# Mingrui-Yu/A-Simple-Stereo-SLAM-System-with-Deep-Loop-Closing

Measured on AMD Instinct MI355X. Metric: stereo frames/sec (ORB+match+LCD+BA-build) @1241x376, higher is better.
Workload: dtype u8/int32 (ORB, Hamming), f32 via f16x3 / bf16x6 split products on the matrix cores with f32 accumulate (CALC conv1 / conv2, DB scan), f64 (triangulation, BA)

## Files before the change

### a-simple-stereo-slam-system-with-deep-loop-closing_amd/csrc/orb_engine.hip

```cpp
#include <math.h>
#include <stdlib.h>
#include <string.h>

#include <vector>

#include "common.h"
#include "orb_plan.h"

namespace myslam_hip {

void launch_resize(const ResizeArgs& a, int batch, hipStream_t s);
void launch_resize_chain(const ResizeArgs* lv, int n, int batch, hipStream_t s);
bool resize_is_little(const ResizeArgs& a, int batch);
int resize_chain_max();
int pyr_head_levels();
void launch_pyr_head(const ResizeArgs* lv, int n, int rows, int cols, uint8_t* dst0, int dpitch0, size_t dstride0, int b0, int batch,
                     uint32_t* p0, int n0, uint32_t* p1, int n1, uint32_t* p2, int n2, uint32_t* p3, int n3, hipStream_t s);
void launch_blur(const BlurArgs& a, int batch, hipStream_t s);
bool blur_uses_strips(const BlurArgs& a);
bool resize_uses_strips(const ResizeArgs& a);
void launch_fast(const OrbPlan& P, const uint8_t* pyr, size_t pyrStride, const uint8_t* maskPyr, uint32_t* cand,
                 int32_t* candCount, const uint32_t* statPrev, uint32_t* statCur, int forceMode, int batch, hipStream_t s);
bool launch_octree(const OrbPlan& P, const uint32_t* cand, const int32_t* candCount, uint32_t* sortbuf, const uint32_t* octTab, uint32_t* selOut,
                   int32_t* selCount, int32_t* status, int batch, uint16_t* order, hipStream_t s, const BlurArgs* blurLv, int nBlur);
bool describe_uses_tile_order(bool have_order, int detectOnly, int batch);
void launch_describe(const OrbPlan& P, const uint8_t* pyr, const uint8_t* blur, size_t pyrStride, const uint32_t* selOut,
                     const int32_t* selCount, myslam_keypoint* kps, uint8_t* desc, int32_t* counts, int32_t* status,
                     int cap, int detectOnly, int batch, uint16_t* order, bool order_ready, int blocks_per_cu, hipStream_t s);
void launch_screen(const OrbPlan& P, const uint8_t* pyr, myslam_keypoint* kin, int n, myslam_keypoint* kout, uint8_t* keep,
                   hipStream_t s);
void launch_calc_desc(const OrbPlan& P, const uint8_t* blur, const myslam_keypoint* kps, int n, uint8_t* desc, hipStream_t s);
void launch_unpack_cands(const uint32_t* cand, int n, int32_t* xs, int32_t* ys, int32_t* sc, hipStream_t s);
void launch_blur_levels(const BlurArgs* lv, int n, int batch, hipStream_t s);
bool blur_mfma_tables(int w, int h, const int q[7], std::vector<uint4>& tab, size_t& offH, size_t& offV);
void blur_mfma_ident(std::vector<uint4>& tab, size_t& offI);
void launch_zero_u32(uint32_t* p0, int n0, uint32_t* p1, int n1, uint32_t* p2, int n2, uint32_t* p3, int n3, hipStream_t s);
void launch_ingest_clear(const uint8_t* src, int rows, int cols, int step, size_t sstride, uint8_t* dst, int dpitch, size_t dstride, int batch,
                         uint32_t* p0, int n0, uint32_t* p1, int n1, uint32_t* p2, int n2, uint32_t* p3, int n3, hipStream_t s);
void launch_ingest(const uint8_t* src, int rows, int cols, int step, size_t sstride, uint8_t* dst, int dpitch,
                   size_t dstride, int batch, hipStream_t s);
// ... 33 lines not shown
    MYSLAM_HIP_CHECK(hipMalloc((void**)&p, n * sizeof(T)));
    return MYSLAM_OK;
}

}

using namespace myslam_hip;

struct myslam_orb {
    int nfeatures, nlevels, iniTh, minTh;
    float scaleFactor;
    std::vector<float> scale, invScale;
    std::vector<int> nPerLevel;
    int umax[16];
    hipStream_t stream = nullptr;
    hipStream_t aux = nullptr;
    hipEvent_t evFork = nullptr, evJoin = nullptr;
    hipEvent_t evUserFast = nullptr;
    hipEvent_t evUserGate = nullptr;

    int rows = 0, cols = 0;
    OrbPlan full{}, det{};

    int batchCap = 0;
    bool maskAlloc = false;
    uint8_t *d_pyr = nullptr, *d_blur = nullptr, *d_mask = nullptr;
    uint32_t* d_cand = nullptr;
    uint32_t* d_sort = nullptr;
    int32_t *d_candCount = nullptr, *d_selCount = nullptr, *d_status = nullptr;
    uint32_t* d_sel = nullptr;
    uint16_t* d_order = nullptr;
    uint32_t* d_octTab = nullptr;
    uint32_t* d_stripTab = nullptr;
    uint32_t* d_fastStat = nullptr; int fastFlip = 0;
    int optFastMode = -1;
    int optInternalStream = 1;
    int optCopyInput = 0;
    int optStopAfter = 0;
    int tapsSet = 0, taps[7] = {0};
    int optSideBlocksPerCu = 0;
    int optBlurMfma = 0;
    uint4* d_blurTab = nullptr; bool blurTabValid = false; size_t blurOffI = 0, blurOffH[MAXL] = {0}, blurOffV[MAXL] = {0}; bool blurLvOk[MAXL] = {false}; int blurVconst = 0;
    int ensure_blur_tables();

    struct HostGraph { hipGraphExec_t exec = nullptr; hipGraph_t graph = nullptr; uint64_t gen = 0; int rows = 0, cols = 0, step = 0, dcap = 0, calls = 0; bool mask = false; };
    HostGraph hostGraph[2][2];
    uint64_t gen = 1;
    struct Clear { uint32_t* p[4]; int n[4]; } clr{{nullptr, nullptr, nullptr, nullptr}, {0, 0, 0, 0}};
    hipStream_t hostStream = nullptr;
    uint8_t* h_pin = nullptr; size_t pinBytes = 0;
    int ensure_pin(size_t bytes);
    void drop_host_graphs();
    uint8_t *d_stageImg = nullptr, *d_stageMask = nullptr; size_t stageImgBytes = 0, stageMaskBytes = 0;
    myslam_keypoint *d_stageKps = nullptr, *d_stageKps2 = nullptr; uint8_t* d_stageDesc = nullptr; uint8_t* d_stageKeep = nullptr;
    int32_t* d_stageCounts = nullptr; int stageCap = 0;
    uint8_t* d_stageOut = nullptr; size_t stageOutBytes = 0, stageDescOff = 0;

    int make_tables();
    int make_plan(int r, int c);
    int ensure(int batch, int r, int c, bool needMask);
    int ensure_stage(size_t imgBytes, size_t maskBytes, int cap);
    int build_pyramids(const uint8_t* d_imgs, int batch, int step, size_t stride, const uint8_t* d_masks, int nlev);
    ResizeArgs level_resize_args(uint8_t* base, int l) const;
    BlurArgs level_blur_args(int l) const;
    int blur_levels(int batch, int nlev, hipStream_t s);
    void fill_blur_args(BlurArgs* lv, int nlev) const;
// ... 109 lines not shown
            const int spr = (g.nCols + 3) / 4;
            for (int strip = 0; strip < g.nRows * spr; strip++) {
                uint32_t* e = st.data() + (size_t)(g.stripBase + strip) * 8;
                const int ci = strip / spr, cj0 = (strip - ci * spr) * 4;
                const int iniY = MIN_BORDER + ci * g.hCell;
                int ncell = 0, pairs = 0; uint32_t wcs = 0; int hr = 0;
                if (iniY < g.maxBY - 3) {
                    hr = std::min(iniY + g.hCell + 6, g.maxBY) - iniY;
                    const int hc = hr - 6;
                    if (hc > 0)
                        for (int c = 0; c < 4; c++) {
                            const int cj = cj0 + c, iniX = MIN_BORDER + cj * g.wCell;
                            int wc = 0;
                            if (cj < g.nCols && iniX < g.maxBX - 6) wc = std::max(0, std::min(iniX + g.wCell + 6, g.maxBX) - iniX - 6);
                            if (wc > 0) ncell = c + 1;
                            wcs |= (uint32_t)wc << (8 * c);
                            pairs += ((wc + 1) >> 1) * hc;
                        }
                }
                if (ncell == 0) wcs = 0;
                e[0] = (uint32_t)l | ((uint32_t)ci << 8) | ((uint32_t)cj0 << 16) | ((uint32_t)ncell << 24);
                e[1] = (uint32_t)iniY | ((uint32_t)hr << 16);
                e[2] = (uint32_t)(MIN_BORDER + cj0 * g.wCell) | ((uint32_t)g.wCell << 16);
                e[3] = wcs; e[4] = (uint32_t)g.pitch; e[5] = (uint32_t)pairs;
                e[6] = (uint32_t)(g.imgOff & 0xffffffffu); e[7] = (uint32_t)(g.imgOff >> 32);
            }
        }
        int rc = dev_alloc(d_stripTab, st.size());
        if (rc) return rc;
        if ((rc = upload_table(d_stripTab, st.data(), st.size() * sizeof(uint32_t)))) return rc;
        P.stripTab = d_stripTab;
    }
    full = P;
    det = P;
    det.nlevels = 1;
    det.ncells = P.lv[0].nCols * P.lv[0].nRows;
    det.nstrips = P.lv[0].nRows * ((P.lv[0].nCols + 3) / 4);
    det.lv[0].N = nfeatures;
    det.lv[0].nodeCap = (std::max(nfeatures + 4, 4 * P.lv[0].nIni + 4) + 3) & ~3;
    if (det.lv[0].nodeCap > 4092) return MYSLAM_ERR_UNSUPPORTED;
    det.lv[0].outBase = 0;
    det.totalOut = det.lv[0].nodeCap;
    rows = r; cols = c;
    return MYSLAM_OK;
}

int myslam_orb::ensure(int batch, int r, int c, bool needMask) {
    if (r != rows || c != cols) {
        MYSLAM_HIP_CHECK(hipStreamSynchronize(stream));
        int rc = make_plan(r, c);
        if (rc) { rows = cols = 0; return rc; }
        batchCap = 0; gen++; blurTabValid = false;
    }
    const int detOut = det.totalOut;
    const size_t selPer = (size_t)std::max(full.totalOut, detOut);
    if (batch > batchCap) {
        MYSLAM_HIP_CHECK(hipStreamSynchronize(stream));
        gen++;
        int rc;
        if ((rc = dev_alloc(d_pyr, (size_t)batch * full.pyrBytes + 64))) return rc;
        if ((rc = dev_alloc(d_blur, (size_t)batch * full.pyrBytes + 4096))) return rc;
        if ((rc = dev_alloc(d_cand, (size_t)batch * full.totalKeyCap))) return rc;
        if ((rc = dev_alloc(d_sort, (size_t)batch * full.totalKeyCap * 2))) return rc;
        if ((rc = dev_alloc(d_candCount, (size_t)batch * MAXL))) return rc;
        if ((rc = dev_alloc(d_selCount, (size_t)batch * MAXL))) return rc;
        if ((rc = dev_alloc(d_status, (size_t)batch))) return rc;
// ... 40 lines not shown
                launch_ingest(src + (size_t)n0 * stride, P.rows, P.cols, step, stride, dst0, P.lv[0].pitch, P.pyrBytes, batch - n0, stream);
            }
        }
        for (; l < nlev;) {
            ScopedProf sp(P_RESIZE, stream);
            ResizeArgs a = level_resize_args(base, l);
            if (l == 1 && n0 > 0) { a.src0 = d_imgs; a.spitch0 = step; a.sstride0 = stride; a.n0 = n0; }
            ResizeArgs grp[4]; int ng = 0;
            const int gmax = resize_chain_max();
            if (gmax > 1 && resize_is_little(a, batch)) {
                static const double kEvals[4] = {1, 5, 21, 85};
                double evals = (double)batch * a.dw * a.dh;
                grp[ng++] = a;
                while (ng < gmax && l + ng < nlev) {
                    const ResizeArgs nx = level_resize_args(base, l + ng);
                    evals += (double)batch * nx.dw * nx.dh * kEvals[ng];
                    if (!resize_is_little(nx, batch) || evals > 6e6) break;
                    grp[ng++] = nx;
                }
            }
            if (ng > 1) { launch_resize_chain(grp, ng, batch, stream); l += ng; }
            else { launch_resize(a, batch, stream); l++; }
        }
    }
    return MYSLAM_OK;
}
ResizeArgs myslam_orb::level_resize_args(uint8_t* base, int l) const {
    const OrbPlan& P = full;
    ResizeArgs a;
    a.src = base + P.lv[l - 1].imgOff; a.sw = P.lv[l - 1].w; a.sh = P.lv[l - 1].h; a.spitch = P.lv[l - 1].pitch; a.sstride = P.pyrBytes;
    a.src0 = nullptr; a.spitch0 = 0; a.n0 = 0; a.sstride0 = 0;
    a.dst = base + P.lv[l].imgOff; a.dw = P.lv[l].w; a.dh = P.lv[l].h; a.dpitch = P.lv[l].pitch; a.dstride = P.pyrBytes;
    a.scale_x = 1. / ((double)a.dw / a.sw); a.scale_y = 1. / ((double)a.dh / a.sh);
    return a;
}
int myslam_orb::ensure_blur_tables() {
    if (blurTabValid) return MYSLAM_OK;
    std::vector<uint4> tab;
    int q[7];
    if (tapsSet) memcpy(q, taps, sizeof(q)); else gauss_q8(0, q);
    int sum = 0;
    for (int t = 0; t < 7; t++) sum += q[t];
    blurVconst = sum * 128 * sum + 32768;
    blur_mfma_ident(tab, blurOffI);
    for (int l = 0; l < full.nlevels; l++) blurLvOk[l] = blur_mfma_tables(full.lv[l].w, full.lv[l].h, q, tab, blurOffH[l], blurOffV[l]);
    MYSLAM_HIP_CHECK(hipStreamSynchronize(stream));
    int rc = dev_alloc(d_blurTab, tab.size());
    if (rc) return rc;
    if ((rc = upload_table(d_blurTab, tab.data(), tab.size() * sizeof(uint4)))) return rc;
    blurTabValid = true; gen++;
    return MYSLAM_OK;
}

BlurArgs myslam_orb::level_blur_args(int l) const {
    const OrbPlan& P = full;
    BlurArgs a;
    a.src = d_pyr + P.lv[l].imgOff; a.dst = d_blur + P.lv[l].imgOff;
    a.w = P.lv[l].w; a.h = P.lv[l].h; a.spitch = a.dpitch = P.lv[l].pitch; a.sstride = a.dstride = P.pyrBytes;
    a.src0 = nullptr; a.spitch0 = 0; a.n0 = 0; a.sstride0 = 0;
    a.dtiled = 1;
    if (tapsSet) memcpy(a.q, taps, sizeof(taps)); else gauss_q8(0, a.q);
    if (optBlurMfma && blurTabValid && blurLvOk[l]) { a.tabH = d_blurTab + blurOffH[l]; a.tabV = d_blurTab + blurOffV[l]; a.ident = d_blurTab + blurOffI; a.vconst = blurVconst; }
    return a;
}
void myslam_orb::fill_blur_args(BlurArgs* lv, int nlev) const {
    const OrbPlan& P = full;
// ... 102 lines not shown
    if (h_pin) { (void)hipHostFree(h_pin); h_pin = nullptr; pinBytes = 0; }
    gen++;
    const size_t want = (bytes + (bytes >> 2) + 4095) & ~(size_t)4095;
    MYSLAM_HIP_CHECK(hipHostMalloc((void**)&h_pin, want));
    pinBytes = want;
    return MYSLAM_OK;
}

void myslam_orb::drop_host_graphs() {
    for (auto& row : hostGraph)
        for (auto& g : row) { if (g.exec) (void)hipGraphExecDestroy(g.exec); if (g.graph) (void)hipGraphDestroy(g.graph); g = HostGraph(); }
}

int myslam_orb::ensure_stage(size_t imgBytes, size_t maskBytes, int cap) {
    if (imgBytes > stageImgBytes) { gen++; int rc = dev_alloc(d_stageImg, imgBytes); if (rc) return rc; stageImgBytes = imgBytes; }
    if (maskBytes > stageMaskBytes) { gen++; int rc = dev_alloc(d_stageMask, maskBytes); if (rc) return rc; stageMaskBytes = maskBytes; }
    if (cap > stageCap) {
        gen++;
        int rc;
        const size_t oK = 256, oD = oK + (((size_t)cap * sizeof(myslam_keypoint) + 255) & ~(size_t)255), total = oD + (size_t)cap * 32;
        if ((rc = dev_alloc(d_stageOut, total))) return rc;
        stageOutBytes = total; stageDescOff = oD;
        d_stageCounts = reinterpret_cast<int32_t*>(d_stageOut);
        d_stageKps = reinterpret_cast<myslam_keypoint*>(d_stageOut + oK);
        d_stageDesc = d_stageOut + oD;
        if ((rc = dev_alloc(d_stageKps2, (size_t)cap))) return rc;
        if ((rc = dev_alloc(d_stageKeep, (size_t)cap))) return rc;
        stageCap = cap;
    }
    return MYSLAM_OK;
}

void myslam_orb::free_all() {
    void* ptrs[] = {d_blurTab, d_fastStat, d_octTab, d_stripTab, d_pyr, d_blur, d_mask, d_cand, d_sort, d_candCount, d_selCount, d_status, d_sel, d_order, d_stageImg, d_stageMask,
                    d_stageOut, d_stageKps2, d_stageKeep};
    for (void* p : ptrs) if (p) (void)hipFree(p);
    if (aux) { (void)hipStreamSynchronize(aux); (void)hipStreamDestroy(aux); (void)hipEventDestroy(evFork); (void)hipEventDestroy(evJoin); aux = nullptr; }
    drop_host_graphs();
    if (hostStream) { (void)hipStreamSynchronize(hostStream); (void)hipStreamDestroy(hostStream); hostStream = nullptr; }
    if (h_pin) { (void)hipHostFree(h_pin); h_pin = nullptr; pinBytes = 0; }
}

extern "C" {

int myslam_orb_create(myslam_orb** out, int nfeatures, float scale_factor, int nlevels, int ini_th_fast, int min_th_fast) {
    if (!out || nfeatures < 1 || nlevels < 1 || nlevels > MAXL || !(scale_factor > 1.0f) || ini_th_fast < 0 ||
        min_th_fast < 1 || min_th_fast > ini_th_fast || ini_th_fast > 255 || scale_factor > 2.5f)
        return MYSLAM_ERR_INVALID;
    int ndev = 0;
    if (hipGetDeviceCount(&ndev) != hipSuccess || ndev < 1) return MYSLAM_ERR_HIP;
    myslam_orb* h = new myslam_orb();
    h->nfeatures = nfeatures; h->scaleFactor = scale_factor; h->nlevels = nlevels; h->iniTh = ini_th_fast; h->minTh = min_th_fast;
    int rc = h->make_tables();
    if (rc) { delete h; return rc; }
    *out = h;
    return MYSLAM_OK;
}

int myslam_orb_destroy(myslam_orb* h) {
    if (!h) return MYSLAM_ERR_INVALID;
    (void)hipStreamSynchronize(h->stream);
    h->free_all();
    delete h;
    return MYSLAM_OK;
}

int myslam_orb_set_stream(myslam_orb* h, void* s) {
// ... 334 lines not shown
```

### a-simple-stereo-slam-system-with-deep-loop-closing_amd/csrc/orb_kernels.hip

```cpp
#include <stdio.h>
#include <stdlib.h>

#include <type_traits>

#include "common.h"
#include "orb_plan.h"

namespace myslam_hip {

typedef unsigned short u16x2 __attribute__((ext_vector_type(2)));

#ifdef MYSLAM_BLOCK_TRACE
__device__ unsigned long long* g_bt_buf = nullptr;
__device__ unsigned int g_bt_cap = 0, g_bt_n = 0;
struct BlockTrace {
    unsigned long long t0 = 0, marks = 0, aux = 0; int kid; unsigned hw = 0; bool on = false;
    __device__ __forceinline__ void mark(int i) {
        if (on) marks |= ((__builtin_amdgcn_s_memrealtime() - t0) & 0xffffull) << (16 * i);
    }
    __device__ __forceinline__ BlockTrace(int kid_) : kid(kid_) {
        if (threadIdx.x != 0 || g_bt_buf == nullptr) return;
        const unsigned xcc = __builtin_amdgcn_s_getreg((3 << 11) | 20) & 0xf;
        if (xcc != 0) return;
        hw = __builtin_amdgcn_s_getreg((31 << 11) | 4);
// ... 113 lines not shown
        return min(max(v, 0), 255);
    }
}

__host__ __device__ constexpr int rc_px(int J) { return J >= 4 ? 1 : 4; }

template <int J>
__device__ __forceinline__ void rc_store(const ResizeChain& c, const uint8_t* S, uint8_t* D, int item) {
    const int dw = c.dw[J - 1], dh = c.dh[J - 1], gpr = (dw + 3) >> 2;
    if constexpr (rc_px(J) == 4) {
        const int dy = item / gpr, dx4 = (item - dy * gpr) * 4;
        if (dy >= dh) return;
        uint32_t packed = 0;
#pragma unroll
        for (int k = 0; k < 4; k++) packed |= (uint32_t)rc_pix<J>(c, S, min(dx4 + k, dw - 1), dy) << (8 * k);
        *reinterpret_cast<uint32_t*>(D + (size_t)dy * c.dpitch[J - 1] + dx4) = packed;
    } else {
        const int dy = item / (4 * gpr), dx = item - dy * 4 * gpr;
        if (dy >= dh) return;
        D[(size_t)dy * c.dpitch[J - 1] + dx] = (uint8_t)rc_pix<J>(c, S, min(dx, dw - 1), dy);
    }
}

__device__ __forceinline__ void rc_block(const ResizeChain& c, int blk, int b) {
    const uint8_t* S = c.src + (size_t)b * c.sstride;
    if (blk < c.blk0[1]) rc_store<1>(c, S, c.dst[0] + (size_t)b * c.dstride, blk * 256 + (int)threadIdx.x);
    else if (blk < c.blk0[2]) rc_store<2>(c, S, c.dst[1] + (size_t)b * c.dstride, (blk - c.blk0[1]) * 256 + (int)threadIdx.x);
    else if (blk < c.blk0[3]) rc_store<3>(c, S, c.dst[2] + (size_t)b * c.dstride, (blk - c.blk0[2]) * 256 + (int)threadIdx.x);
    else rc_store<4>(c, S, c.dst[3] + (size_t)b * c.dstride, (blk - c.blk0[3]) * 256 + (int)threadIdx.x);
}

__global__ __launch_bounds__(256) void k_resize_chain(ResizeChain c) { rc_block(c, blockIdx.x, blockIdx.y); }

constexpr int RS_R = 8;
constexpr int RS_NB = 2;
constexpr int RS_MAXR = 12;

__global__ __launch_bounds__(256) void k_resize_strip(ResizeArgs a, int nstrips, int nbands) {
    MYSLAM_SIDE_PRIO();
    MYSLAM_BT(1);
    const int lane = threadIdx.x & 63;
    const int wid = __builtin_amdgcn_readfirstlane((int)(blockIdx.x * 4 + (threadIdx.x >> 6)));
    const int ngroups = (nbands + RS_NB - 1) / RS_NB;
    if (wid >= nstrips * ngroups) return;
    const int strip = wid % nstrips, group = wid / nstrips;
    const int b = blockIdx.z;
    const int dx4 = strip * 256 + 4 * lane;
    const bool has = dx4 < a.dw;
    const bool ext = b < a.n0;
    const uint8_t* src = ext ? a.src0 + (size_t)b * a.sstride0 : a.src + (size_t)b * a.sstride;
    const int spitch = ext ? a.spitch0 : a.spitch;
    uint8_t* dst = a.dst + (size_t)b * a.dstride;
    int sx[4]; uint32_t aw[4];
#pragma unroll
    for (int k = 0; k < 4; k++) {
        int c0, c1;
        resize_coord(min(dx4 + k, a.dw - 1), a.scale_x, a.sw, true, sx[k], c0, c1);
        aw[k] = (uint32_t)c0 | ((uint32_t)c1 << 16);
    }
    uint32_t selk[4];
#pragma unroll
    for (int k = 0; k < 4; k++) { const uint32_t o = (uint32_t)(sx[k] - sx[0]); selk[k] = 0x0c000c00u | ((o + 1u) << 16) | o; }
    const int gy0 = group * RS_NB * RS_R;
    int ysy, yb0, yb1;
    resize_coord(min(gy0 + (lane & (RS_NB * RS_R - 1)), a.dh - 1), a.scale_y, a.sh, false, ysy, yb0, yb1);
    for (int bi = 0; bi < RS_NB; bi++) {
        const int dy0 = gy0 + bi * RS_R, dy1 = min(dy0 + RS_R, a.dh), l0 = bi * RS_R;
        if (dy0 >= a.dh) break;
        const int rfirst = min(max(__builtin_amdgcn_readlane(ysy, l0), 0), a.sh - 1);
        const int rlast = min(max(__builtin_amdgcn_readlane(ysy, l0 + dy1 - 1 - dy0) + 1, 0), a.sh - 1);
        const int nrows = rlast - rfirst + 1;
        uint2 raw8[RS_MAXR];
        if (ext) {
#pragma unroll
            for (int rr = 0; rr < RS_MAXR; rr++) {
                const uint8_t* row = src + (size_t)(rfirst + min(rr, nrows - 1)) * spitch;
                raw8[rr] = make_uint2(0u, 0u);
                if (has && rr < nrows) __builtin_memcpy(&raw8[rr], row + sx[0], 8);
            }
        } else {
            uint32_t raw12[RS_MAXR][3];
            const uint32_t xal = (uint32_t)sx[0] & ~3u, sh = (uint32_t)sx[0] & 3u;
#pragma unroll
            for (int rr = 0; rr < RS_MAXR; rr++) {
                const uint8_t* row = src + (size_t)(rfirst + min(rr, nrows - 1)) * spitch;
                raw12[rr][0] = raw12[rr][1] = raw12[rr][2] = 0u;
                if (has && rr < nrows) __builtin_memcpy(raw12[rr], __builtin_assume_aligned(row + xal, 4), 12);
            }
#pragma unroll
            for (int rr = 0; rr < RS_MAXR; rr++)
                raw8[rr] = make_uint2(__builtin_amdgcn_alignbyte(raw12[rr][1], raw12[rr][0], sh), __builtin_amdgcn_alignbyte(raw12[rr][2], raw12[rr][1], sh));
        }
        uint32_t raw[RS_MAXR][4];
#pragma unroll
        for (int rr = 0; rr < RS_MAXR; rr++) {
            if (rr >= RS_R + 1 && rr >= nrows) {
#pragma unroll
                for (int k = 0; k < 4; k++) raw[rr][k] = 0u;
                continue;
            }
#pragma unroll
            for (int k = 0; k < 4; k++) {
                const uint32_t pp = __builtin_amdgcn_perm(raw8[rr].y, raw8[rr].x, selk[k]);
                raw[rr][k] = __builtin_amdgcn_udot2(__builtin_bit_cast(u16x2, pp), __builtin_bit_cast(u16x2, aw[k]), 0u, false) & ~15u;
            }
        }
        int dy = dy0;
        int sy = __builtin_amdgcn_readlane(ysy, l0);
        uint32_t b0 = (uint32_t)__builtin_amdgcn_readlane(yb0, l0) << 12, b1 = (uint32_t)__builtin_amdgcn_readlane(yb1, l0) << 12;
#pragma unroll
        for (int rr = 0; rr < RS_MAXR; rr++) {
            while (dy < dy1 && min(max(sy, 0), a.sh - 1) - rfirst == rr) {
                const bool same = min(max(sy + 1, 0), a.sh - 1) - rfirst == rr;
                uint32_t packed = 0;
#pragma unroll
                for (int k = 0; k < 4; k++) {
                    const uint32_t tA = raw[rr][k], tB = same ? raw[rr][k] : raw[rr + 1 < RS_MAXR ? rr + 1 : rr][k];
                    uint32_t hA, hB;
                    asm("v_mul_hi_u32_u24 %0, %1, %2" : "=v"(hA) : "s"(b0), "v"(tA));
                    asm("v_mul_hi_u32_u24 %0, %1, %2" : "=v"(hB) : "s"(b1), "v"(tB));
                    const uint32_t v = (hA + hB + 2u) >> 2;
                    packed |= v << (8 * k);
                }
                if (has) *reinterpret_cast<uint32_t*>(dst + (size_t)dy * a.dpitch + dx4) = packed;
                dy++;
                if (dy < dy1) {
                    sy = __builtin_amdgcn_readlane(ysy, l0 + dy - dy0);
                    b0 = (uint32_t)__builtin_amdgcn_readlane(yb0, l0 + dy - dy0) << 12; b1 = (uint32_t)__builtin_amdgcn_readlane(yb1, l0 + dy - dy0) << 12;
                }
            }
        }
    }
}

__device__ __forceinline__ int reflect101(int p, int len) {
    if (len == 1) return 0;
    while (p < 0 || p >= len) p = (p < 0) ? -p : 2 * len - 2 - p;
    return p;
}

__device__ __forceinline__ uint32_t pack4_sat_hi16(uint32_t s0, uint32_t s1, uint32_t s2, uint32_t s3) {
    uint32_t p01 = __builtin_amdgcn_perm(s1, s0, 0x07060302u), p23 = __builtin_amdgcn_perm(s3, s2, 0x07060302u), u01, u23;
    asm("v_sat_pk_u8_i16 %0, %1" : "=v"(u01) : "v"(p01));
    asm("v_sat_pk_u8_i16 %0, %1" : "=v"(u23) : "v"(p23));
    return (u01 & 0xffffu) | (u23 << 16);
}

constexpr int B2_W = 128, B2_H = 32, B2_IH = B2_H + 6, B2_IP = B2_W + 8, B2_IDW = B2_IP / 4, B2_PR = B2_IH / 2;

__global__ __launch_bounds__(256) void k_blur7_dot(BlurArgs a) {
    __shared__ __attribute__((aligned(16))) uint8_t s_in[B2_IH * B2_IP];
    __shared__ __attribute__((aligned(16))) uint32_t s_hp[B2_PR * B2_W];
    const int t = threadIdx.x;
    const int b = blockIdx.z;
    const int x0 = blockIdx.x * B2_W, y0 = blockIdx.y * B2_H;
    const uint8_t* src = a.src + (size_t)b * a.sstride;
    const bool aligned = ((a.spitch & 3) == 0) && ((reinterpret_cast<uintptr_t>(src) & 3) == 0);
    const int nout = min(B2_H, a.h - y0);
    const int nrp = (nout + 6 + 1) >> 1;
    for (int i = t; i < 2 * nrp * B2_IDW; i += 256) {
        const int r = i / B2_IDW, k = i - r * B2_IDW;
        const int gy = reflect101(y0 + r - 3, a.h);
        const int gx = x0 - 4 + 4 * k;
        const uint8_t* row = src + (size_t)gy * a.spitch;
        uint32_t v;
// ... 2182 lines not shown
    if (b < g.b0) return;
    const int ib = blk - c.blk0[RC_MAX];
    ingest_part(g.src, g.rows, g.cols, g.step, g.sstride, g.dst, g.dpitch, g.dstride, g.tpr, g.rpb, ib % g.gx, ib / g.gx, b);
}

__global__ __launch_bounds__(256) void k_zero_u32(ZeroArgs a) {
    const int i = blockIdx.x * 256 + threadIdx.x;
#pragma unroll
    for (int k = 0; k < 4; k++)
        if (a.p[k] && i < a.n[k]) a.p[k][i] = 0u;
}
void launch_zero_u32(uint32_t* p0, int n0, uint32_t* p1, int n1, uint32_t* p2, int n2, uint32_t* p3, int n3, hipStream_t s) {
    ZeroArgs a{{p0, p1, p2, p3}, {n0, n1, n2, n3}};
    const int n = max(max(n0, n1), max(n2, n3));
    if (n > 0) hipLaunchKernelGGL(k_zero_u32, dim3((n + 255) / 256), dim3(256), 0, s, a);
}

static void ingest_launch(const uint8_t* src, int rows, int cols, int step, size_t sstride, uint8_t* dst, int dpitch,
                          size_t dstride, int batch, const ZeroArgs& z, hipStream_t s) {
    const int t = (cols + 15) / 16;
    const int tpr = t < 256 ? t : 256, rpb = t < 256 ? 256 / t : 1;
    dim3 grid((t + 255) / 256, (rows + rpb - 1) / rpb, batch);
    hipLaunchKernelGGL(k_ingest, grid, dim3(256), 0, s, src, rows, cols, step, sstride, dst, dpitch, dstride, tpr, rpb, z);
}
void launch_ingest(const uint8_t* src, int rows, int cols, int step, size_t sstride, uint8_t* dst, int dpitch,
                   size_t dstride, int batch, hipStream_t s) {
    ingest_launch(src, rows, cols, step, sstride, dst, dpitch, dstride, batch, ZeroArgs{{nullptr, nullptr, nullptr, nullptr}, {0, 0, 0, 0}}, s);
}
void launch_ingest_clear(const uint8_t* src, int rows, int cols, int step, size_t sstride, uint8_t* dst, int dpitch, size_t dstride, int batch,
                         uint32_t* p0, int n0, uint32_t* p1, int n1, uint32_t* p2, int n2, uint32_t* p3, int n3, hipStream_t s) {
    ingest_launch(src, rows, cols, step, sstride, dst, dpitch, dstride, batch, ZeroArgs{{p0, p1, p2, p3}, {n0, n1, n2, n3}}, s);
}

bool resize_uses_strips(const ResizeArgs& a) { return (double)RS_R * a.scale_y + 2.0 <= (double)RS_MAXR && a.scale_x <= 1.6; }

bool resize_is_little(const ResizeArgs& a, int batch) { return a.n0 == 0 && (size_t)batch * a.dw * a.dh < (size_t)1500000; }

#ifndef MYSLAM_RESIZE_CHAIN_MAX
#define MYSLAM_RESIZE_CHAIN_MAX 3
#endif
int resize_chain_max() { return MYSLAM_RESIZE_CHAIN_MAX < RC_MAX ? MYSLAM_RESIZE_CHAIN_MAX : RC_MAX; }

static ResizeChain make_chain(const ResizeArgs* lv, int n) {
    ResizeChain c;
    c.src = lv[0].src; c.sw = lv[0].sw; c.sh = lv[0].sh; c.spitch = lv[0].spitch; c.sstride = lv[0].sstride;
    c.n = n; c.dstride = lv[0].dstride; c.blk0[0] = 0;
    for (int j = 0; j < RC_MAX; j++) {
        const ResizeArgs& a = lv[j < n ? j : n - 1];
        c.dst[j] = a.dst; c.dw[j] = a.dw; c.dh[j] = a.dh; c.dpitch[j] = a.dpitch; c.scale_x[j] = a.scale_x; c.scale_y[j] = a.scale_y;
        c.blk0[j + 1] = c.blk0[j] + (j < n ? (((a.dw + 3) / 4) * (4 / rc_px(j + 1)) * a.dh + 255) / 256 : 0);
    }
    return c;
}
void launch_resize_chain(const ResizeArgs* lv, int n, int batch, hipStream_t s) {
    const ResizeChain c = make_chain(lv, n);
    hipLaunchKernelGGL(k_resize_chain, dim3(c.blk0[RC_MAX], batch), dim3(256), 0, s, c);
}
void launch_pyr_head(const ResizeArgs* lv, int n, int rows, int cols, uint8_t* dst0, int dpitch0, size_t dstride0, int b0, int batch,
                     uint32_t* p0, int n0, uint32_t* p1, int n1, uint32_t* p2, int n2, uint32_t* p3, int n3, hipStream_t s) {
    const ResizeChain c = make_chain(lv, n);
    const int t = (cols + 15) / 16;
    IngestPart g{lv[0].src, rows, cols, lv[0].spitch, lv[0].sstride, dst0, dpitch0, dstride0, t < 256 ? t : 256, t < 256 ? 256 / t : 1, (t + 255) / 256, b0};
    const int iblocks = g.gx * ((rows + g.rpb - 1) / g.rpb);
    hipLaunchKernelGGL(k_pyr_head, dim3(c.blk0[RC_MAX] + iblocks, batch), dim3(256), 0, s, c, g, ZeroArgs{{p0, p1, p2, p3}, {n0, n1, n2, n3}});
}
#ifndef MYSLAM_PYR_HEAD_LEVELS
#define MYSLAM_PYR_HEAD_LEVELS 2
#endif
int pyr_head_levels() { return MYSLAM_PYR_HEAD_LEVELS < 3 ? MYSLAM_PYR_HEAD_LEVELS : 3; }

void launch_resize(const ResizeArgs& a, int batch, hipStream_t s) {
    const bool little = resize_is_little(a, batch);
    if (resize_uses_strips(a) && !little) {
        const int nstrips = (a.dw + 255) / 256, nbands = (a.dh + RS_R - 1) / RS_R;
        const int ngroups = (nbands + RS_NB - 1) / RS_NB;
        hipLaunchKernelGGL(k_resize_strip, dim3((nstrips * ngroups + 3) / 4, 1, batch), dim3(256), 0, s, a, nstrips, nbands);
        return;
    }
    dim3 grid((a.dw + 255) / 256, (a.dh + 3) / 4, batch);
    hipLaunchKernelGGL(k_resize, grid, dim3(256), 0, s, a);
}

bool blur_uses_strips(const BlurArgs& a) {
    return a.w >= 8 && a.h >= 8 && (a.spitch & 3) == 0 && ((reinterpret_cast<uintptr_t>(a.src) | a.sstride) & 3) == 0;
}

void launch_blur_levels(const BlurArgs* lv, int n, int batch, hipStream_t s) {
    BlurMulti M; M.n = 0; M.wave0[0] = 0;
    BlurMfmaMulti X; X.n = 0; X.wave0[0] = 0;
    for (int i = 0; i < n; i++) {
        const BlurArgs& a = lv[i];
        if (a.tabH && a.tabV && a.ident && a.dtiled && (a.dpitch & 15) == 0 && ((reinterpret_cast<uintptr_t>(a.dst) | a.dstride) & 15) == 0) {
            X.a[X.n] = a; X.tabHOff[X.n] = 0; X.tabVOff[X.n] = 0; X.wave0[X.n + 1] = X.wave0[X.n] + (a.w + 31) / 32; X.n++;
        } else if (blur_uses_strips(a)) {
            const int nstrips = (a.w + 255) / 256, nbands = (a.h + B3_R - 1) / B3_R;
            M.a[M.n] = a; M.nstrips[M.n] = nstrips; M.wave0[M.n + 1] = M.wave0[M.n] + nstrips * nbands; M.n++;
        } else {
            dim3 grid((a.w + B2_W - 1) / B2_W, (a.h + B2_H - 1) / B2_H, batch);
            hipLaunchKernelGGL(k_blur7_dot, grid, dim3(256), 0, s, a);
        }
    }
    if (M.n) hipLaunchKernelGGL(k_blur7_strip, dim3((M.wave0[M.n] + 3) / 4, 1, batch), dim3(256), 0, s, M);
    if (X.n) hipLaunchKernelGGL(k_blur7_mfma, dim3((X.wave0[X.n] + 3) / 4, 1, batch), dim3(256), 0, s, X);
}
void launch_blur(const BlurArgs& a, int batch, hipStream_t s) { launch_blur_levels(&a, 1, batch, s); }

#ifndef MYSLAM_BLUR_WITH_OCTREE
#define MYSLAM_BLUR_WITH_OCTREE 1
#endif
// ... 100 lines not shown
```

### a-simple-stereo-slam-system-with-deep-loop-closing_amd/csrc/orb_plan.h

```cpp
#pragma once
#include <stddef.h>
#include <stdint.h>

namespace myslam_hip {

constexpr int MAXL = 12;
constexpr int EDGE_THRESHOLD = 19;
constexpr int MIN_BORDER = 16;
constexpr int PATCH_SIZE = 31;
constexpr int HALF_PATCH = 15;
constexpr int MAX_CELL = 59;
constexpr int MAX_DEPTH = 13;
constexpr int ROOT_SHIFT = 26;

struct LevelGeom {
    int w, h, pitch;
    int nCols, nRows, wCell, hCell;
    int maxBX, maxBY;
    int cellBase;
    int stripBase;
    int N;
    int nIni;
    float hX;
    int sortDepth;
    int ndepth;
    int keyCap;
    int nodeCap;
    int outBase;
    float scale;
    float scaledPatch;
    size_t imgOff;
    size_t keyOff;
    int tabOff, tabX, tabY;
};

struct OrbPlan {
    int nlevels;
    int rows, cols;
    int ncells;
    int nstrips;
    int iniTh, minTh;
    int totalKeyCap;
    int totalOut;
    size_t pyrBytes;
    const uint8_t* ext0; size_t ext0Stride; int ext0Pitch, ext0N;
    int stripBaseOf[MAXL];
    const uint32_t* stripTab;
    LevelGeom lv[MAXL];
};

struct ResizeArgs {
    const uint8_t* src; int sw, sh, spitch; size_t sstride;
    const uint8_t* src0 = nullptr; int spitch0 = 0, n0 = 0; size_t sstride0 = 0;
    uint8_t* dst; int dw, dh, dpitch; size_t dstride;
    double scale_x, scale_y;
};

struct BlurArgs {
    const uint8_t* src; uint8_t* dst; int w, h, spitch, dpitch; size_t sstride, dstride;
    const uint8_t* src0 = nullptr; int spitch0 = 0, n0 = 0; size_t sstride0 = 0;
    int q[7];
    int dtiled = 0;
    const uint4* tabH = nullptr; const uint4* tabV = nullptr; const uint4* ident = nullptr; int vconst = 0;
};

__host__ __device__ inline size_t tiled_off(int x, int y, int pitch) {
    return (size_t)(y >> 3) * (size_t)pitch * 8 + (size_t)((x >> 4) << 7) + (size_t)(((y & 7) << 4) | (x & 15));
}

}
```

Baseline: 80800.

## Rewrite strip resize as a streaming row walk using precomputed coordinate tables

Bilinear pyramid resize coordinates and weights for columns and rows are now precomputed on the host per level and uploaded as tables. The strip kernel loads these tables instead of recomputing them. Each wave now walks a tall band of 64 output rows, streaming source rows through a small prefetch ring and reusing each horizontally filtered row for consecutive outputs. This replaces the old fixed 8-row bands that reloaded overlapping rows and used large register arrays. It narrows the scale range that qualifies for the strip path, exposes fewer waves per level, and aborts if tables are missing.

```diff
diff --git a/a-simple-stereo-slam-system-with-deep-loop-closing_amd/csrc/orb_engine.hip b/a-simple-stereo-slam-system-with-deep-loop-closing_amd/csrc/orb_engine.hip
--- a/a-simple-stereo-slam-system-with-deep-loop-closing_amd/csrc/orb_engine.hip
+++ b/a-simple-stereo-slam-system-with-deep-loop-closing_amd/csrc/orb_engine.hip
@@ -6,6 +6,7 @@
 
 #include "common.h"
 #include "orb_plan.h"
+#include "resize_tab.h"
 
 namespace myslam_hip {
 
@@ -105,6 +106,8 @@
     uint16_t* d_order = nullptr;
     uint32_t* d_octTab = nullptr;
     uint32_t* d_stripTab = nullptr;
+    uint32_t* d_resizeTab = nullptr;
+    size_t resizeColOff[MAXL] = {0}, resizeRowOff[MAXL] = {0}; bool resizeLvOk[MAXL] = {false};
     uint32_t* d_fastStat = nullptr; int fastFlip = 0;
     int optFastMode = -1;
     int optInternalStream = 1;
@@ -280,6 +283,25 @@
         P.stripTab = d_stripTab;
     }
     full = P;
+    {
+        std::vector<uint32_t> rt;
+        std::vector<ResizeColRec> cr; std::vector<ResizeRowRec> rr;
+        for (int l = 1; l < nlevels; l++) {
+            const ResizeArgs a = level_resize_args(nullptr, l);
+            resizeLvOk[l] = resize_uses_strips(a);
+            if (!resizeLvOk[l]) continue;
+            resize_col_records(a.sw, a.dw, a.scale_x, (a.dw + 255) / 256 * 64, cr);
+            resize_row_records(a.sh, a.dh, a.scale_y, rr);
+            resizeColOff[l] = rt.size();
+            rt.insert(rt.end(), reinterpret_cast<const uint32_t*>(cr.data()), reinterpret_cast<const uint32_t*>(cr.data() + cr.size()));
+            resizeRowOff[l] = rt.size();
+            rt.insert(rt.end(), reinterpret_cast<const uint32_t*>(rr.data()), reinterpret_cast<const uint32_t*>(rr.data() + rr.size()));
+            rt.resize((rt.size() + 7) & ~(size_t)7, 0u);
+        }
+        int rc = dev_alloc(d_resizeTab, rt.size());
+        if (rc) return rc;
+        if (!rt.empty() && (rc = upload_table(d_resizeTab, rt.data(), rt.size() * sizeof(uint32_t)))) return rc;
+    }
     det = P;
     det.nlevels = 1;
     det.ncells = P.lv[0].nCols * P.lv[0].nRows;
@@ -386,6 +408,7 @@
     a.src0 = nullptr; a.spitch0 = 0; a.n0 = 0; a.sstride0 = 0;
     a.dst = base + P.lv[l].imgOff; a.dw = P.lv[l].w; a.dh = P.lv[l].h; a.dpitch = P.lv[l].pitch; a.dstride = P.pyrBytes;
     a.scale_x = 1. / ((double)a.dw / a.sw); a.scale_y = 1. / ((double)a.dh / a.sh);
+    if (d_resizeTab && resizeLvOk[l]) { a.colTab = d_resizeTab + resizeColOff[l]; a.rowTab = d_resizeTab + resizeRowOff[l]; }
     return a;
 }
 int myslam_orb::ensure_blur_tables() {
@@ -554,7 +577,7 @@
 }
 
 void myslam_orb::free_all() {
-    void* ptrs[] = {d_blurTab, d_fastStat, d_octTab, d_stripTab, d_pyr, d_blur, d_mask, d_cand, d_sort, d_candCount, d_selCount, d_status, d_sel, d_order, d_stageImg, d_stageMask,
+    void* ptrs[] = {d_blurTab, d_fastStat, d_octTab, d_stripTab, d_resizeTab, d_pyr, d_blur, d_mask, d_cand, d_sort, d_candCount, d_selCount, d_status, d_sel, d_order, d_stageImg, d_stageMask,
                     d_stageOut, d_stageKps2, d_stageKeep};
     for (void* p : ptrs) if (p) (void)hipFree(p);
     if (aux) { (void)hipStreamSynchronize(aux); (void)hipStreamDestroy(aux); (void)hipEventDestroy(evFork); (void)hipEventDestroy(evJoin); aux = nullptr; }
diff --git a/a-simple-stereo-slam-system-with-deep-loop-closing_amd/csrc/orb_kernels.hip b/a-simple-stereo-slam-system-with-deep-loop-closing_amd/csrc/orb_kernels.hip
--- a/a-simple-stereo-slam-system-with-deep-loop-closing_amd/csrc/orb_kernels.hip
+++ b/a-simple-stereo-slam-system-with-deep-loop-closing_amd/csrc/orb_kernels.hip
@@ -169,105 +169,102 @@
 
 __global__ __launch_bounds__(256) void k_resize_chain(ResizeChain c) { rc_block(c, blockIdx.x, blockIdx.y); }
 
-constexpr int RS_R = 8;
-constexpr int RS_NB = 2;
-constexpr int RS_MAXR = 12;
-
-__global__ __launch_bounds__(256) void k_resize_strip(ResizeArgs a, int nstrips, int nbands) {
+#ifndef MYSLAM_RS_BAND
+#define MYSLAM_RS_BAND 64
+#endif
+#ifndef MYSLAM_RS_PF
+#define MYSLAM_RS_PF 4
+#endif
+constexpr int RS_BAND = MYSLAM_RS_BAND;
+constexpr int RS_PF = MYSLAM_RS_PF;
+
+typedef uint32_t rs_u32x3 __attribute__((ext_vector_type(3)));
+typedef uint32_t rs_u32x2 __attribute__((ext_vector_type(2)));
+
+template <bool EXT>
+__device__ __forceinline__ void resize_strip_walk(const ResizeArgs& a, const uint8_t* src, int spitch, uint8_t* dst, int lane, int strip, int dy0, int dy1) {
+    typedef const uint32_t __attribute__((address_space(4))) * ConstU32;
+    typedef const uint8_t __attribute__((address_space(1))) * GlobalU8;
+    typedef std::conditional_t<EXT, rs_u32x2, rs_u32x3> Raw;
+    typedef Raw __attribute__((aligned(EXT ? 1 : 4))) RawMem;
+    const int dx4 = strip * 256 + 4 * lane;
+    const uint4* crec = reinterpret_cast<const uint4*>(a.colTab) + 2 * (size_t)(strip * 64 + lane);
+    const uint4 c0 = crec[0], c1 = crec[1];
+    const uint32_t sel[4] = {0x0c010c00u, c0.y, c0.z, c0.w}, aw[4] = {c1.x, c1.y, c1.z, c1.w};
+    const uint32_t xoff = EXT ? c0.x : (c0.x & ~3u), bsh = c0.x & 3u;
+    const ConstU32 rt = (ConstU32)((uintptr_t)a.rowTab);
+    const int r0 = (int)rt[4 * dy0];
+    const int rlast = min((int)rt[4 * (dy1 - 1)] + 1, a.sh - 1);
+    auto load_row = [&](int r) -> Raw {
+        uintptr_t rp = (uintptr_t)src + (size_t)min(r, rlast) * (size_t)spitch;
+        uint32_t xo = xoff;
+        asm("" : "+s"(rp));
+        asm volatile("" : "+v"(xo));
+        return *reinterpret_cast<const RawMem __attribute__((address_space(1)))*>((GlobalU8)rp + xo);
+    };
+    auto hrow = [&](const Raw& w, uint32_t* h) {
+        uint32_t x, y;
+        if constexpr (EXT) { x = w.x; y = w.y; }
+        else { x = __builtin_amdgcn_alignbyte(w.y, w.x, bsh); y = __builtin_amdgcn_alignbyte(w.z, w.y, bsh); }
+#pragma unroll
+        for (int k = 0; k < 4; k++) {
+            const uint32_t pp = __builtin_amdgcn_perm(y, x, sel[k]);
+            h[k] = __builtin_amdgcn_udot2(__builtin_bit_cast(u16x2, pp), __builtin_bit_cast(u16x2, aw[k]), 0u, false) & ~15u;
+        }
+    };
+    auto emit = [&](int dy, uint32_t b0, uint32_t b1, const uint32_t* tA, const uint32_t* tB) {
+        uint32_t packed = 0;
+#pragma unroll
+        for (int k = 0; k < 4; k++) {
+            uint32_t hA, hB;
+            asm("v_mul_hi_u32_u24 %0, %1, %2" : "=v"(hA) : "s"(b0), "v"(tA[k]));
+            asm("v_mul_hi_u32_u24 %0, %1, %2" : "=v"(hB) : "s"(b1), "v"(tB[k]));
+            const uint32_t v = (hA + hB + 2u) >> 2;
+            packed |= v << (8 * k);
+        }
+        uintptr_t dp = (uintptr_t)dst + (size_t)dy * (size_t)a.dpitch;
+        uint32_t xd = (uint32_t)dx4;
+        asm("" : "+s"(dp));
+        asm volatile("" : "+v"(xd));
+        *reinterpret_cast<uint32_t __attribute__((address_space(1)))*>((uint8_t __attribute__((address_space(1)))*)dp + xd) = packed;
+    };
+    Raw ring[RS_PF];
+#pragma unroll
+    for (int u = 0; u < RS_PF; u++) ring[u] = load_row(r0 + u);
+    int dy = dy0;
+    uint32_t cs = rt[4 * dy], cb0 = rt[4 * dy + 2], cb1 = rt[4 * dy + 3];
+    uint32_t ns = rt[4 * dy + 4], nb0 = rt[4 * dy + 6], nb1 = rt[4 * dy + 7];
+    uint32_t hA[4] = {0u, 0u, 0u, 0u}, hB[4];
+    for (int base = 0; r0 + base <= rlast + 1; base += RS_PF) {
+#pragma unroll
+        for (int u = 0; u < RS_PF; u++) {
+            hrow(ring[u], hB);
+            ring[u] = load_row(r0 + base + u + RS_PF);
+            if ((int)cs == r0 + base + u - 1) {
+                emit(dy, cb0, cb1, hA, hB);
+                if (++dy >= dy1) return;
+                cs = ns; cb0 = nb0; cb1 = nb1;
+                ns = rt[4 * dy + 4]; nb0 = rt[4 * dy + 6]; nb1 = rt[4 * dy + 7];
+            }
+#pragma unroll
+            for (int k = 0; k < 4; k++) hA[k] = hB[k];
+        }
+    }
+}
+
+__global__ __launch_bounds__(256) void k_resize_strip(ResizeArgs a, int nstrips, int nbands, int band) {
     MYSLAM_SIDE_PRIO();
     MYSLAM_BT(1);
     const int lane = threadIdx.x & 63;
     const int wid = __builtin_amdgcn_readfirstlane((int)(blockIdx.x * 4 + (threadIdx.x >> 6)));
-    const int ngroups = (nbands + RS_NB - 1) / RS_NB;
-    if (wid >= nstrips * ngroups) return;
-    const int strip = wid % nstrips, group = wid / nstrips;
+    if (wid >= nstrips * nbands) return;
+    const int strip = wid % nstrips, bi = wid / nstrips;
     const int b = blockIdx.z;
-    const int dx4 = strip * 256 + 4 * lane;
-    const bool has = dx4 < a.dw;
-    const bool ext = b < a.n0;
-    const uint8_t* src = ext ? a.src0 + (size_t)b * a.sstride0 : a.src + (size_t)b * a.sstride;
-    const int spitch = ext ? a.spitch0 : a.spitch;
+    const int dy0 = bi * band, dy1 = min(dy0 + band, a.dh);
+    if (strip * 256 + 4 * lane >= a.dw) return;
     uint8_t* dst = a.dst + (size_t)b * a.dstride;
-    int sx[4]; uint32_t aw[4];
-#pragma unroll
-    for (int k = 0; k < 4; k++) {
-        int c0, c1;
-        resize_coord(min(dx4 + k, a.dw - 1), a.scale_x, a.sw, true, sx[k], c0, c1);
-        aw[k] = (uint32_t)c0 | ((uint32_t)c1 << 16);
-    }
-    uint32_t selk[4];
-#pragma unroll
-    for (int k = 0; k < 4; k++) { const uint32_t o = (uint32_t)(sx[k] - sx[0]); selk[k] = 0x0c000c00u | ((o + 1u) << 16) | o; }
-    const int gy0 = group * RS_NB * RS_R;
-    int ysy, yb0, yb1;
-    resize_coord(min(gy0 + (lane & (RS_NB * RS_R - 1)), a.dh - 1), a.scale_y, a.sh, false, ysy, yb0, yb1);
-    for (int bi = 0; bi < RS_NB; bi++) {
-        const int dy0 = gy0 + bi * RS_R, dy1 = min(dy0 + RS_R, a.dh), l0 = bi * RS_R;
-        if (dy0 >= a.dh) break;
-        const int rfirst = min(max(__builtin_amdgcn_readlane(ysy, l0), 0), a.sh - 1);
-        const int rlast = min(max(__builtin_amdgcn_readlane(ysy, l0 + dy1 - 1 - dy0) + 1, 0), a.sh - 1);
-        const int nrows = rlast - rfirst + 1;
-        uint2 raw8[RS_MAXR];
-        if (ext) {
-#pragma unroll
-            for (int rr = 0; rr < RS_MAXR; rr++) {
-                const uint8_t* row = src + (size_t)(rfirst + min(rr, nrows - 1)) * spitch;
-                raw8[rr] = make_uint2(0u, 0u);
-                if (has && rr < nrows) __builtin_memcpy(&raw8[rr], row + sx[0], 8);
-            }
-        } else {
-            uint32_t raw12[RS_MAXR][3];
-            const uint32_t xal = (uint32_t)sx[0] & ~3u, sh = (uint32_t)sx[0] & 3u;
-#pragma unroll
-            for (int rr = 0; rr < RS_MAXR; rr++) {
-                const uint8_t* row = src + (size_t)(rfirst + min(rr, nrows - 1)) * spitch;
-                raw12[rr][0] = raw12[rr][1] = raw12[rr][2] = 0u;
-                if (has && rr < nrows) __builtin_memcpy(raw12[rr], __builtin_assume_aligned(row + xal, 4), 12);
-            }
-#pragma unroll
-            for (int rr = 0; rr < RS_MAXR; rr++)
-                raw8[rr] = make_uint2(__builtin_amdgcn_alignbyte(raw12[rr][1], raw12[rr][0], sh), __builtin_amdgcn_alignbyte(raw12[rr][2], raw12[rr][1], sh));
-        }
-        uint32_t raw[RS_MAXR][4];
-#pragma unroll
-        for (int rr = 0; rr < RS_MAXR; rr++) {
-            if (rr >= RS_R + 1 && rr >= nrows) {
-#pragma unroll
-                for (int k = 0; k < 4; k++) raw[rr][k] = 0u;
-                continue;
-            }
-#pragma unroll
-            for (int k = 0; k < 4; k++) {
-                const uint32_t pp = __builtin_amdgcn_perm(raw8[rr].y, raw8[rr].x, selk[k]);
-                raw[rr][k] = __builtin_amdgcn_udot2(__builtin_bit_cast(u16x2, pp), __builtin_bit_cast(u16x2, aw[k]), 0u, false) & ~15u;
-            }
-        }
-        int dy = dy0;
-        int sy = __builtin_amdgcn_readlane(ysy, l0);
-        uint32_t b0 = (uint32_t)__builtin_amdgcn_readlane(yb0, l0) << 12, b1 = (uint32_t)__builtin_amdgcn_readlane(yb1, l0) << 12;
-#pragma unroll
-        for (int rr = 0; rr < RS_MAXR; rr++) {
-            while (dy < dy1 && min(max(sy, 0), a.sh - 1) - rfirst == rr) {
-                const bool same = min(max(sy + 1, 0), a.sh - 1) - rfirst == rr;
-                uint32_t packed = 0;
-#pragma unroll
-                for (int k = 0; k < 4; k++) {
-                    const uint32_t tA = raw[rr][k], tB = same ? raw[rr][k] : raw[rr + 1 < RS_MAXR ? rr + 1 : rr][k];
-                    uint32_t hA, hB;
-                    asm("v_mul_hi_u32_u24 %0, %1, %2" : "=v"(hA) : "s"(b0), "v"(tA));
-                    asm("v_mul_hi_u32_u24 %0, %1, %2" : "=v"(hB) : "s"(b1), "v"(tB));
-                    const uint32_t v = (hA + hB + 2u) >> 2;
-                    packed |= v << (8 * k);
-                }
-                if (has) *reinterpret_cast<uint32_t*>(dst + (size_t)dy * a.dpitch + dx4) = packed;
-                dy++;
-                if (dy < dy1) {
-                    sy = __builtin_amdgcn_readlane(ysy, l0 + dy - dy0);
-                    b0 = (uint32_t)__builtin_amdgcn_readlane(yb0, l0 + dy - dy0) << 12; b1 = (uint32_t)__builtin_amdgcn_readlane(yb1, l0 + dy - dy0) << 12;
-                }
-            }
-        }
-    }
+    if (b < a.n0) resize_strip_walk<true>(a, a.src0 + (size_t)b * a.sstride0, a.spitch0, dst, lane, strip, dy0, dy1);
+    else resize_strip_walk<false>(a, a.src + (size_t)b * a.sstride, a.spitch, dst, lane, strip, dy0, dy1);
 }
 
 __device__ __forceinline__ int reflect101(int p, int len) {
@@ -2516,7 +2513,7 @@
     ingest_launch(src, rows, cols, step, sstride, dst, dpitch, dstride, batch, ZeroArgs{{p0, p1, p2, p3}, {n0, n1, n2, n3}}, s);
 }
 
-bool resize_uses_strips(const ResizeArgs& a) { return (double)RS_R * a.scale_y + 2.0 <= (double)RS_MAXR && a.scale_x <= 1.6; }
+bool resize_uses_strips(const ResizeArgs& a) { return a.scale_y >= 1.0 && a.scale_y <= 1.25 && a.scale_x <= 1.6; }
 
 bool resize_is_little(const ResizeArgs& a, int batch) { return a.n0 == 0 && (size_t)batch * a.dw * a.dh < (size_t)1500000; }
 
@@ -2556,9 +2553,9 @@
 void launch_resize(const ResizeArgs& a, int batch, hipStream_t s) {
     const bool little = resize_is_little(a, batch);
     if (resize_uses_strips(a) && !little) {
-        const int nstrips = (a.dw + 255) / 256, nbands = (a.dh + RS_R - 1) / RS_R;
-        const int ngroups = (nbands + RS_NB - 1) / RS_NB;
-        hipLaunchKernelGGL(k_resize_strip, dim3((nstrips * ngroups + 3) / 4, 1, batch), dim3(256), 0, s, a, nstrips, nbands);
+        if (!a.colTab || !a.rowTab) { fprintf(stderr, "myslam_hip: launch_resize: the plan holds no resize tables for this level\n"); abort(); }
+        const int nstrips = (a.dw + 255) / 256, band = RS_BAND, nbands = (a.dh + band - 1) / band;
+        hipLaunchKernelGGL(k_resize_strip, dim3((nstrips * nbands + 3) / 4, 1, batch), dim3(256), 0, s, a, nstrips, nbands, band);
         return;
     }
     dim3 grid((a.dw + 255) / 256, (a.dh + 3) / 4, batch);
diff --git a/a-simple-stereo-slam-system-with-deep-loop-closing_amd/csrc/orb_plan.h b/a-simple-stereo-slam-system-with-deep-loop-closing_amd/csrc/orb_plan.h
--- a/a-simple-stereo-slam-system-with-deep-loop-closing_amd/csrc/orb_plan.h
+++ b/a-simple-stereo-slam-system-with-deep-loop-closing_amd/csrc/orb_plan.h
@@ -54,6 +54,7 @@
     const uint8_t* src0 = nullptr; int spitch0 = 0, n0 = 0; size_t sstride0 = 0;
     uint8_t* dst; int dw, dh, dpitch; size_t dstride;
     double scale_x, scale_y;
+    const uint32_t* colTab = nullptr; const uint32_t* rowTab = nullptr;
 };
 
 struct BlurArgs {
diff --git a/a-simple-stereo-slam-system-with-deep-loop-closing_amd/csrc/resize_tab.h b/a-simple-stereo-slam-system-with-deep-loop-closing_amd/csrc/resize_tab.h
--- /dev/null
+++ b/a-simple-stereo-slam-system-with-deep-loop-closing_amd/csrc/resize_tab.h
@@ -0,0 +1,66 @@
+#pragma once
+#include <math.h>
+#include <stddef.h>
+#include <stdint.h>
+
+#include <algorithm>
+#include <vector>
+
+namespace myslam_hip {
+
+struct ResizeColRec { uint32_t sx0, sel[3], aw[4]; };
+struct ResizeRowRec { uint32_t srow, same, b0, b1; };
+static_assert(sizeof(ResizeColRec) == 32 && sizeof(ResizeRowRec) == 16, "the kernel loads the records as 2 x 16 and 1 x 16 bytes");
+constexpr int RESIZE_ROW_SPARE = 2;
+
+#if defined(__clang__)
+#define MYSLAM_NO_CONTRACT _Pragma("clang fp contract(off)")
+#define MYSLAM_NO_CONTRACT_ATTR
+#else
+#define MYSLAM_NO_CONTRACT
+#define MYSLAM_NO_CONTRACT_ATTR __attribute__((optimize("fp-contract=off")))
+#endif
+MYSLAM_NO_CONTRACT_ATTR inline void resize_coord_host(int d, double scale, int ssize, bool is_x, int& s, int& c0, int& c1) {
+    MYSLAM_NO_CONTRACT
+    const double m = ((double)d + 0.5) * scale;
+    const double e = m - 0.5;
+    float f = (float)e;
+    int si = (int)floorf(f);
+    f = f - (float)si;
+    if (is_x) {
+        if (si < 0) { f = 0.f; si = 0; }
+        if (si >= ssize - 1) { f = 0.f; si = ssize - 1; }
+    }
+    s = si;
+    const float w0 = (1.f - f) * 2048.f, w1 = f * 2048.f;
+    c0 = (int)nearbyintf(w0);
+    c1 = (int)nearbyintf(w1);
+}
+
+inline void resize_col_records(int sw, int dw, double scale_x, int ngroups, std::vector<ResizeColRec>& out) {
+    out.resize((size_t)ngroups);
+    for (int g = 0; g < ngroups; g++) {
+        int sx[4], a0, a1;
+        ResizeColRec& r = out[(size_t)g];
+        for (int k = 0; k < 4; k++) {
+            resize_coord_host(std::min(4 * g + k, dw - 1), scale_x, sw, true, sx[k], a0, a1);
+            r.aw[k] = (uint32_t)a0 | ((uint32_t)a1 << 16);
+            const uint32_t o = (uint32_t)(sx[k] - sx[0]);
+            if (k > 0) r.sel[k - 1] = 0x0c000c00u | ((o + 1u) << 16) | o;
+        }
+        r.sx0 = (uint32_t)sx[0];
+    }
+}
+
+inline void resize_row_records(int sh, int dh, double scale_y, std::vector<ResizeRowRec>& out) {
+    out.resize((size_t)dh + RESIZE_ROW_SPARE);
+    for (int d = 0; d < dh; d++) {
+        int sy, b0, b1;
+        resize_coord_host(d, scale_y, sh, false, sy, b0, b1);
+        const int r0 = std::min(std::max(sy, 0), sh - 1), r1 = std::min(std::max(sy + 1, 0), sh - 1);
+        out[(size_t)d] = ResizeRowRec{(uint32_t)r0, r0 == r1 ? 1u : 0u, (uint32_t)b0 << 12, (uint32_t)b1 << 12};
+    }
+    for (int d = dh; d < dh + RESIZE_ROW_SPARE; d++) out[(size_t)d] = out[(size_t)dh - 1];
+}
+
+}
```

Measured after the change: 84910 (median of 6 runs). +5.1%, better.
